# lxa9867/ImageFolder

Hardware: NVIDIA H100
Metric: tokenizer_train_images_per_sec_256x256 (higher is better)
Workload: dtype bf16

## Files before the change

imagefolder_b200/csrc/attn_kernel.cu:

```cuda
#include "xq_common.cuh"
#include "xq_tc.cuh"

namespace xq {
using namespace xqtc;

constexpr int AT_BM = 128;
constexpr int AT_BN = 128;
constexpr int AT_D = 64;
constexpr int AT_NS = 2;
constexpr int AT_TILE = AT_BM * AT_D * 2;
constexpr int AT_THREADS = 288;

struct AttnFwdSmem {
    static constexpr int Q = 0;
    static constexpr int K = AT_TILE;
    static constexpr int V = AT_TILE * (1 + AT_NS);
    static constexpr int BAR = AT_TILE * (1 + 2 * AT_NS);
    static constexpr int BYTES = BAR + 256;
};

__device__ __forceinline__ void named_bar_sync(int id, int nthreads) { asm volatile("bar.sync %0, %1;" ::"r"(id), "r"(nthreads) : "memory"); }

template <typename E>
__global__ void __launch_bounds__(AT_THREADS, 1)
attn_fwd_kernel(const __grid_constant__ CUtensorMap tmQKV, typename E::T *__restrict__ out, float *__restrict__ lse2, int N, int H,
                int nQ , float c ) {
    extern __shared__ uint8_t smem_raw[];
    uint8_t *base = (uint8_t *)(((uintptr_t)smem_raw + 1023) & ~(uintptr_t)1023);
    uint64_t *bars = (uint64_t *)(base + AttnFwdSmem::BAR);
    uint64_t *q_full = bars + 0;
    uint64_t *k_full = bars + 1;
    uint64_t *k_empty = bars + 1 + AT_NS;
    uint64_t *v_full = bars + 1 + 2 * AT_NS;
    uint64_t *v_empty = bars + 1 + 3 * AT_NS;

    const int tid = threadIdx.x, warp = tid >> 5, lane = tid & 31;
    const int nK = (N + AT_BN - 1) / AT_BN;
    const int bh = blockIdx.x / nQ, qt = blockIdx.x - bh * nQ;
    const int b = bh / H, h = bh - b * H;

    if (tid == 0) {
        mbar_init(q_full, 1);
        for (int i = 0; i < AT_NS; ++i) { mbar_init(&k_full[i], 1); mbar_init(&k_empty[i], 8); mbar_init(&v_full[i], 1); mbar_init(&v_empty[i], 8); }
        mbar_fence_init();
    }
    __syncthreads();

    if (warp == 8) {
        const int colQ = h * AT_D, colK = (H + h) * AT_D, colV = (2 * H + h) * AT_D;
        if (elect_one()) {
            tma_prefetch_desc(&tmQKV);
            mbar_expect_tx(q_full, AT_TILE);
            tma_load_3d(base + AttnFwdSmem::Q, &tmQKV, colQ, qt * AT_BM, b, q_full);
        }
        __syncwarp();
        for (int j = 0; j < nK; ++j) {
            const int st = j % AT_NS;
            const uint32_t ph = ((j / AT_NS) & 1) ^ 1;
            mbar_wait(&k_empty[st], ph);
            if (elect_one()) {
                mbar_expect_tx(&k_full[st], AT_TILE);
                tma_load_3d(base + AttnFwdSmem::K + st * AT_TILE, &tmQKV, colK, j * AT_BN, b, &k_full[st]);
            }
            __syncwarp();
            mbar_wait(&v_empty[st], ph);
            if (elect_one()) {
                mbar_expect_tx(&v_full[st], AT_TILE);
                tma_load_3d(base + AttnFwdSmem::V + st * AT_TILE, &tmQKV, colV, j * AT_BN, b, &v_full[st]);
            }
            __syncwarp();
        }
        return;
    }

    const int wg = warp >> 2, wq = warp & 3;
    const int rq = wg * 64 + wq * 16 + (lane >> 2), cq = 2 * (lane & 3);
    const uint64_t qd = desc_k_sw128(smem_u32(base + AttnFwdSmem::Q + wg * (AT_TILE / 2)));
    float m[2] = {-CUDART_INF_F, -CUDART_INF_F}, l[2] = {0.f, 0.f};
    float o[32];
#pragma unroll
    for (int i = 0; i < 32; ++i) o[i] = 0.f;
    mbar_wait(q_full, 0);
    for (int j = 0; j < nK; ++j) {
        const int st = j % AT_NS;
        const uint32_t ph = (j / AT_NS) & 1;
        float s[64];
        mbar_wait(&k_full[st], ph);
        const uint64_t kd = desc_k_sw128(smem_u32(base + AttnFwdSmem::K + st * AT_TILE));
        wgmma_fence();
#pragma unroll
        for (int k = 0; k < AT_D / 16; ++k) wgmma_m64n128k16_ss<E, 0, 0>(s, desc_adv(qd, k * 32), desc_adv(kd, k * 32), (uint32_t)k);
        wgmma_commit();
        wgmma_wait<0>();
        fence_regs(s);
        __syncwarp();
        if (lane == 0) mbar_arrive(&k_empty[st]);
        const int nv = N - j * AT_BN;
        if (nv < AT_BN) {
#pragma unroll
            for (int i = 0; i < 64; ++i)
                if (8 * (i >> 2) + cq + (i & 1) >= nv) s[i] = -CUDART_INF_F;
        }
        float mx[2] = {m[0], m[1]};
#pragma unroll
        for (int i = 0; i < 64; ++i) mx[(i >> 1) & 1] = fmaxf(mx[(i >> 1) & 1], s[i]);
#pragma unroll
        for (int hh = 0; hh < 2; ++hh) {
            mx[hh] = fmaxf(mx[hh], __shfl_xor_sync(0xffffffffu, mx[hh], 1));
            mx[hh] = fmaxf(mx[hh], __shfl_xor_sync(0xffffffffu, mx[hh], 2));
        }
        float alpha[2], mc[2];
#pragma unroll
        for (int hh = 0; hh < 2; ++hh) {
            alpha[hh] = ex2_approx((m[hh] - mx[hh]) * c);
            m[hh] = mx[hh];
            mc[hh] = mx[hh] * c;
            l[hh] *= alpha[hh];
        }
#pragma unroll
        for (int i = 0; i < 32; ++i) o[i] *= alpha[(i >> 1) & 1];
        uint32_t pa[AT_BN / 16][4];
#pragma unroll
        for (int i = 0; i < 64; i += 2) {
            const int hh = (i >> 1) & 1;
            const float p0 = ex2_approx(fmaf(s[i], c, -mc[hh])), p1 = ex2_approx(fmaf(s[i + 1], c, -mc[hh]));
            l[hh] += p0 + p1;
            pa[i >> 3][((i >> 2) & 1) * 2 + hh] = E::pack(p0, p1);
        }
        mbar_wait(&v_full[st], ph);
        const uint64_t vd = desc_mn_sw128(smem_u32(base + AttnFwdSmem::V + st * AT_TILE), AT_TILE);
        wgmma_fence();
#pragma unroll
        for (int k = 0; k < AT_BN / 16; ++k) wgmma_m64n64k16_rs<E, 1>(o, pa[k], desc_adv(vd, k * 2048), 1u);
        wgmma_commit();
        wgmma_wait<0>();
        fence_regs(o);
        __syncwarp();
        if (lane == 0) mbar_arrive(&v_empty[st]);
    }
#pragma unroll
    for (int hh = 0; hh < 2; ++hh) {
        l[hh] += __shfl_xor_sync(0xffffffffu, l[hh], 1);
        l[hh] += __shfl_xor_sync(0xffffffffu, l[hh], 2);
    }
#pragma unroll
    for (int hh = 0; hh < 2; ++hh) {
        const int n = qt * AT_BM + rq + 8 * hh;
        if (n >= N) continue;
        const float inv = 1.0f / l[hh];
        if (cq == 0) lse2[(size_t)bh * N + n] = fmaf(m[hh], c, log2f(l[hh]));
        typename E::T *orow = out + ((size_t)b * N + n) * H * AT_D + h * AT_D;
#pragma unroll
        for (int jj = 0; jj < AT_D / 8; ++jj)
            *reinterpret_cast<uint32_t *>(orow + 8 * jj + cq) = E::pack(o[4 * jj + 2 * hh] * inv, o[4 * jj + 2 * hh + 1] * inv);
    }
}

constexpr int AB_THREADS = 288;
constexpr int AB_BQ = 64;
constexpr int AB_QS = 3;
constexpr int AB_QTILE = AB_BQ * AT_D * 2;

struct AttnBwdSmem {
    static constexpr int K = 0;
    static constexpr int V = AT_TILE;
    static constexpr int Q = 2 * AT_TILE;
    static constexpr int DO = Q + AB_QS * AB_QTILE;
    static constexpr int DS = DO + AB_QS * AB_QTILE;
    static constexpr int STAT = DS + 2 * AB_QTILE;
    static constexpr int BAR = STAT + AB_QS * 512;
    static constexpr int BYTES = BAR + 256;
};

template <typename E>
__device__ __forceinline__ void bwd_epilogue_frag(const float (&acc)[32], float mul, typename E::T *__restrict__ row0,
                                                  size_t row_stride, bool ok0, bool ok1, float *__restrict__ g_bias_cols, int lane) {
    const int cq = 2 * (lane & 3);
#pragma unroll
    for (int jj = 0; jj < AT_D / 8; ++jj) {
        const uint32_t w0 = E::pack(acc[4 * jj] * mul, acc[4 * jj + 1] * mul);
        const uint32_t w1 = E::pack(acc[4 * jj + 2] * mul, acc[4 * jj + 3] * mul);
        if (ok0) *reinterpret_cast<uint32_t *>(row0 + 8 * jj + cq) = w0;
        if (ok1) *reinterpret_cast<uint32_t *>(row0 + 8 * row_stride + 8 * jj + cq) = w1;
        if (g_bias_cols) {
            float s0 = E::lo(w0) + E::lo(w1);
            float s1 = E::hi(w0) + E::hi(w1);
#pragma unroll
            for (int o = 4; o < 32; o <<= 1) {
                s0 += __shfl_xor_sync(0xffffffffu, s0, o);
                s1 += __shfl_xor_sync(0xffffffffu, s1, o);
            }
            if (lane < 4) {
                atomicAdd(g_bias_cols + 8 * jj + cq, s0);
                atomicAdd(g_bias_cols + 8 * jj + cq + 1, s1);
            }
        }
    }
}

template <typename E>
__global__ void __launch_bounds__(AB_THREADS, 1)
attn_bwd_kernel(const __grid_constant__ CUtensorMap tmQKV, const __grid_constant__ CUtensorMap tmDO, const float *__restrict__ lseP,
                const float *__restrict__ deltaP, float *__restrict__ dq_acc, typename E::T *__restrict__ dqkv, float *__restrict__ g_bias,
                int N, int H, int Npad, float c, float scale) {
    extern __shared__ uint8_t smem_raw[];
    uint8_t *base = (uint8_t *)(((uintptr_t)smem_raw + 1023) & ~(uintptr_t)1023);
    uint64_t *bars = (uint64_t *)(base + AttnBwdSmem::BAR);
    uint64_t *kv_full = bars;
    uint64_t *q_full = bars + 1;
    uint64_t *q_empty = bars + 1 + AB_QS;
    float *s_lse = (float *)(base + AttnBwdSmem::STAT);
    float *s_delta = s_lse + AB_QS * AB_BQ;

    const int tid = threadIdx.x, warp = tid >> 5, lane = tid & 31;
    const int bh = blockIdx.y, b = bh / H, h = bh - b * H;
    const int k0 = blockIdx.x * AT_BN;
    const int colQ = h * AT_D, colK = (H + h) * AT_D, colV = (2 * H + h) * AT_D;
    const int nQ = (N + AB_BQ - 1) / AB_BQ;

    if (tid == 0) {
        mbar_init(kv_full, 1);
        for (int i = 0; i < AB_QS; ++i) { mbar_init(&q_full[i], 1); mbar_init(&q_empty[i], 8); }
        mbar_fence_init();
    }
    __syncthreads();

    if (warp == 8) {
        if (elect_one()) {
            tma_prefetch_desc(&tmQKV);
            tma_prefetch_desc(&tmDO);
            mbar_expect_tx(kv_full, 2 * AT_TILE);
            for (int hf = 0; hf < 2; ++hf) {
                tma_load_3d(base + AttnBwdSmem::K + hf * AB_QTILE, &tmQKV, colK, k0 + hf * AB_BQ, b, kv_full);
                tma_load_3d(base + AttnBwdSmem::V + hf * AB_QTILE, &tmQKV, colV, k0 + hf * AB_BQ, b, kv_full);
            }
        }
        __syncwarp();
        for (int i = 0; i < nQ; ++i) {
            const int st = i % AB_QS;
            mbar_wait(&q_empty[st], ((i / AB_QS) & 1) ^ 1);
            if (elect_one()) {
                mbar_expect_tx(&q_full[st], 2 * AB_QTILE + 2 * AB_BQ * 4);
                tma_load_3d(base + AttnBwdSmem::Q + st * AB_QTILE, &tmQKV, colQ, i * AB_BQ, b, &q_full[st]);
                tma_load_3d(base + AttnBwdSmem::DO + st * AB_QTILE, &tmDO, h * AT_D, i * AB_BQ, b, &q_full[st]);
                bulk_g2s(s_lse + st * AB_BQ, lseP + (size_t)bh * Npad + i * AB_BQ, AB_BQ * 4, &q_full[st]);
                bulk_g2s(s_delta + st * AB_BQ, deltaP + (size_t)bh * Npad + i * AB_BQ, AB_BQ * 4, &q_full[st]);
            }
            __syncwarp();
        }
        return;
    }

    const int wg = warp >> 2, wq = warp & 3;
    const int rq = wq * 16 + (lane >> 2), cq = 2 * (lane & 3);
    const int key0 = k0 + wg * 64 + rq;
    const bool kok0 = key0 < N, kok1 = key0 + 8 < N;
    const uint32_t kw = smem_u32(base + AttnBwdSmem::K + wg * AB_QTILE), vw = smem_u32(base + AttnBwdSmem::V + wg * AB_QTILE);
    const uint64_t kd_k = desc_k_sw128(kw), vd_k = desc_k_sw128(vw), kd_mn = desc_mn_sw128(kw, AT_TILE);
    const uint32_t dsw = smem_u32(base + AttnBwdSmem::DS + wg * AB_QTILE);
    const uint64_t dsd = desc_mn_sw128(dsw, AT_TILE);
    float dv[32], dk[32];
#pragma unroll
    for (int i = 0; i < 32; ++i) dv[i] = dk[i] = 0.f;
    mbar_wait(kv_full, 0);
    for (int i = 0; i < nQ; ++i) {
        const int st = i % AB_QS;
        mbar_wait(&q_full[st], (i / AB_QS) & 1);
        const uint32_t qa = smem_u32(base + AttnBwdSmem::Q + st * AB_QTILE), da = smem_u32(base + AttnBwdSmem::DO + st * AB_QTILE);
        float s[32], dp[32];
        wgmma_fence();
#pragma unroll
        for (int k = 0; k < AT_D / 16; ++k) wgmma_m64n64k16_ss<E, 0, 0>(s, desc_adv(kd_k, k * 32), desc_adv(desc_k_sw128(qa), k * 32), (uint32_t)k);
#pragma unroll
        for (int k = 0; k < AT_D / 16; ++k) wgmma_m64n64k16_ss<E, 0, 0>(dp, desc_adv(vd_k, k * 32), desc_adv(desc_k_sw128(da), k * 32), (uint32_t)k);
        wgmma_commit();
        wgmma_wait<0>();
        fence_regs(s);
        fence_regs(dp);
        const float *L = s_lse + st * AB_BQ, *D = s_delta + st * AB_BQ;
        uint32_t pa[4][4], sa[4][4];
#pragma unroll
        for (int jj = 0; jj < AB_BQ / 8; ++jj) {
            const float2 Lq = *reinterpret_cast<const float2 *>(L + 8 * jj + cq);
            const float2 Dq = *reinterpret_cast<const float2 *>(D + 8 * jj + cq);
#pragma unroll
            for (int hh = 0; hh < 2; ++hh) {
                const bool ok = hh ? kok1 : kok0;
                const float p0 = ok ? ex2_approx(fmaf(s[4 * jj + 2 * hh], c, -Lq.x)) : 0.f;
                const float p1 = ok ? ex2_approx(fmaf(s[4 * jj + 2 * hh + 1], c, -Lq.y)) : 0.f;
                const uint32_t pw = E::pack(p0, p1);
                const float d0 = E::lo(pw) * (dp[4 * jj + 2 * hh] - Dq.x);
                const float d1 = E::hi(pw) * (dp[4 * jj + 2 * hh + 1] - Dq.y);
                const uint32_t dw = E::pack(d0, d1);
                pa[jj >> 1][(jj & 1) * 2 + hh] = pw;
                sa[jj >> 1][(jj & 1) * 2 + hh] = dw;
                asm volatile("st.shared.b32 [%0], %1;" ::"r"(dsw + rowtile_off_bf16(rq + 8 * hh, 8 * jj + cq)), "r"(dw) : "memory");
            }
        }
        fence_async_smem();
        named_bar_sync(1 + wg, 128);
        const uint64_t qd_mn = desc_mn_sw128(qa, AT_TILE), dd_mn = desc_mn_sw128(da, AT_TILE);
        float dq[32];
        wgmma_fence();
#pragma unroll
        for (int k = 0; k < AB_BQ / 16; ++k) {
            wgmma_m64n64k16_rs<E, 1>(dv, pa[k], desc_adv(dd_mn, k * 2048), 1u);
            wgmma_m64n64k16_rs<E, 1>(dk, sa[k], desc_adv(qd_mn, k * 2048), 1u);
        }
#pragma unroll
        for (int k = 0; k < 64 / 16; ++k) wgmma_m64n64k16_ss<E, 1, 1>(dq, desc_adv(dsd, k * 2048), desc_adv(kd_mn, k * 2048), (uint32_t)k);
        wgmma_commit();
        wgmma_wait<0>();
        fence_regs(dv);
        fence_regs(dk);
        fence_regs(dq);
        __syncwarp();
        if (lane == 0) mbar_arrive(&q_empty[st]);
        named_bar_sync(1 + wg, 128);
#pragma unroll
        for (int hh = 0; hh < 2; ++hh) {
            const int q = i * AB_BQ + rq + 8 * hh;
            if (q < N) {
                float *dst = dq_acc + ((size_t)bh * N + q) * AT_D + cq;
#pragma unroll
                for (int jj = 0; jj < AT_D / 8; ++jj)
                    atomicAdd(reinterpret_cast<float2 *>(dst + 8 * jj), make_float2(dq[4 * jj + 2 * hh], dq[4 * jj + 2 * hh + 1]));
            }
        }
    }
    const size_t W = (size_t)3 * H * AT_D;
    typename E::T *row = dqkv + ((size_t)b * N + key0) * W;
    bwd_epilogue_frag<E>(dv, 1.0f, row + colV, W, kok0, kok1, g_bias ? g_bias + colV : nullptr, lane);
    bwd_epilogue_frag<E>(dk, scale, row + colK, W, kok0, kok1, g_bias ? g_bias + colK : nullptr, lane);
}


constexpr int AB_KTAIL_MAX = 4;
constexpr int AB_PREP_ROWS = 128;

template <typename E>
__device__ __forceinline__ void unpack8(const uint4 &w, float (&f)[8]) {
    const uint32_t x[4] = {w.x, w.y, w.z, w.w};
#pragma unroll
    for (int e = 0; e < 4; ++e) { f[2 * e] = E::lo(x[e]); f[2 * e + 1] = E::hi(x[e]); }
}

template <typename E, int NT>
__global__ void __launch_bounds__(256, 2)
attn_bwd_prep_kernel(const typename E::T *__restrict__ qkv, const typename E::T *__restrict__ out, const typename E::T *__restrict__ dout,
                     const float *__restrict__ lse2, float *__restrict__ lseP, float *__restrict__ deltaP, float *__restrict__ dq_acc,
                     float *__restrict__ dsT, typename E::T *__restrict__ dqkv, float *__restrict__ g_bias, int N, int H, int Npad,
                     float c, float scale) {
    constexpr int NTA = NT > 0 ? NT : 1;
    __shared__ float red[NT > 0 ? 8 : 1][2][NTA][AT_D];
    __shared__ __align__(16) float skv[2][NTA][AT_D];
    const int bh = blockIdx.y, b = bh / H, h = bh - b * H;
    const int lane = threadIdx.x & 31, sub = threadIdx.x & 7, rloc = threadIdx.x >> 3;
    const int n0 = N - NT;
    const size_t W = (size_t)3 * H * AT_D;
    const typename E::T *qb = qkv + (size_t)b * N * W + h * AT_D + sub * 8;
    const size_t ob = (size_t)b * N * H * AT_D + h * AT_D + sub * 8;
    float aK[NTA][8], aV[NTA][8];
    if constexpr (NT > 0) {
        if (threadIdx.x < NT * 16) {
            const int t = threadIdx.x >> 4, isv = (threadIdx.x >> 3) & 1;
            float f[8];
            unpack8<E>(*reinterpret_cast<const uint4 *>(qb + (size_t)(n0 + t) * W + (size_t)(1 + isv) * H * AT_D), f);
#pragma unroll
            for (int e = 0; e < 8; ++e) skv[isv][t][sub * 8 + e] = f[e];
        }
#pragma unroll
        for (int t = 0; t < NT; ++t) {
#pragma unroll
            for (int e = 0; e < 8; ++e) aK[t][e] = aV[t][e] = 0.f;
        }
        __syncthreads();
    }
    constexpr int PASSES = AB_PREP_ROWS / 32;
    extern __shared__ uint4 prep_stage[];
    auto prefetch = [&](int blk, int stg) {
#pragma unroll
        for (int ps = 0; ps < PASSES; ++ps) {
            const int n = blk * AB_PREP_ROWS + ps * 32 + rloc;
            const int nc = n < N ? n : N - 1;
            uint4 *dst = prep_stage + ((size_t)(stg * 3) * PASSES + ps) * 256 + threadIdx.x;
            cp_async16(dst, out + ob + (size_t)nc * H * AT_D);
            cp_async16(dst + PASSES * 256, dout + ob + (size_t)nc * H * AT_D);
            cp_async16(dst + 2 * PASSES * 256, qb + (size_t)nc * W);
        }
        cp_async_commit();
    };
    if constexpr (NT > 0) prefetch(blockIdx.x, 0);
    int stg = 0;
    for (int blk = blockIdx.x; blk * AB_PREP_ROWS < Npad; blk += gridDim.x, stg ^= 1) {
        uint4 ow[PASSES], gw[PASSES], qw[PASSES];
        float lq[PASSES];
#pragma unroll
        for (int ps = 0; ps < PASSES; ++ps) {
            const int n = blk * AB_PREP_ROWS + ps * 32 + rloc;
            const int nc = n < N ? n : N - 1;
            if constexpr (NT == 0) {
                ow[ps] = *reinterpret_cast<const uint4 *>(out + ob + (size_t)nc * H * AT_D);
                gw[ps] = *reinterpret_cast<const uint4 *>(dout + ob + (size_t)nc * H * AT_D);
            }
            lq[ps] = lse2[(size_t)bh * N + nc];
        }
        if constexpr (NT > 0) {
            if ((blk + (int)gridDim.x) * AB_PREP_ROWS < Npad) { prefetch(blk + gridDim.x, stg ^ 1); cp_async_wait<1>(); }
            else cp_async_wait<0>();
        }
#pragma unroll
        for (int ps = 0; ps < PASSES; ++ps) {
            const int n = blk * AB_PREP_ROWS + ps * 32 + rloc;
            const bool live = n < N;
            float ov[8], gv[8];
            if constexpr (NT > 0) {
                const uint4 *src = prep_stage + ((size_t)(stg * 3) * PASSES + ps) * 256 + threadIdx.x;
                ow[ps] = src[0];
                gw[ps] = src[PASSES * 256];
                qw[ps] = src[2 * PASSES * 256];
            }
            unpack8<E>(ow[ps], ov);
            unpack8<E>(gw[ps], gv);
            float dl = 0.f;
#pragma unroll
            for (int e = 0; e < 8; ++e) dl = fmaf(ov[e], gv[e], dl);
            dl += __shfl_xor_sync(0xffffffffu, dl, 1);
            dl += __shfl_xor_sync(0xffffffffu, dl, 2);
            dl += __shfl_xor_sync(0xffffffffu, dl, 4);
            if (!live) dl = 0.f;
            if (sub == 0) {
                deltaP[(size_t)bh * Npad + n] = dl;
                lseP[(size_t)bh * Npad + n] = live ? lq[ps] : CUDART_INF_F;
            }
            if (live) {
                float4 *z = reinterpret_cast<float4 *>(dq_acc + ((size_t)bh * N + n) * AT_D + sub * 8);
                z[0] = make_float4(0.f, 0.f, 0.f, 0.f);
                z[1] = make_float4(0.f, 0.f, 0.f, 0.f);
            }
            if constexpr (NT > 0) {
                float qv[8];
                unpack8<E>(qw[ps], qv);
#pragma unroll
                for (int t = 0; t < NT; ++t) {
                    float sx = 0.f, pd = 0.f;
                    const float4 k0 = *reinterpret_cast<const float4 *>(&skv[0][t][sub * 8]), k1 = *reinterpret_cast<const float4 *>(&skv[0][t][sub * 8 + 4]);
                    const float4 v0 = *reinterpret_cast<const float4 *>(&skv[1][t][sub * 8]), v1 = *reinterpret_cast<const float4 *>(&skv[1][t][sub * 8 + 4]);
                    const float kt[8] = {k0.x, k0.y, k0.z, k0.w, k1.x, k1.y, k1.z, k1.w}, vt[8] = {v0.x, v0.y, v0.z, v0.w, v1.x, v1.y, v1.z, v1.w};
#pragma unroll
                    for (int e = 0; e < 8; ++e) { sx = fmaf(qv[e], kt[e], sx); pd = fmaf(gv[e], vt[e], pd); }
#pragma unroll
                    for (int o = 4; o > 0; o >>= 1) {
                        sx += __shfl_xor_sync(0xffffffffu, sx, o);
                        pd += __shfl_xor_sync(0xffffffffu, pd, o);
                    }
                    const float p = live ? ex2_approx(fmaf(sx, c, -lq[ps])) : 0.f;
                    const float ds = p * (pd - dl);
#pragma unroll
                    for (int e = 0; e < 8; ++e) { aV[t][e] = fmaf(p, gv[e], aV[t][e]); aK[t][e] = fmaf(ds, qv[e], aK[t][e]); }
                    if (sub == 0 && live) dsT[((size_t)bh * N + n) * NT + t] = ds;
                }
            }
        }
    }
    if constexpr (NT > 0) {
        const int warp = threadIdx.x >> 5;
#pragma unroll
        for (int t = 0; t < NT; ++t) {
#pragma unroll
            for (int e = 0; e < 8; ++e) {
                float a = aK[t][e], v = aV[t][e];
                a += __shfl_xor_sync(0xffffffffu, a, 8);  v += __shfl_xor_sync(0xffffffffu, v, 8);
                a += __shfl_xor_sync(0xffffffffu, a, 16); v += __shfl_xor_sync(0xffffffffu, v, 16);
                if (lane < 8) { red[warp][0][t][sub * 8 + e] = a; red[warp][1][t][sub * 8 + e] = v; }
            }
        }
        __syncthreads();
        if (threadIdx.x < 2 * AT_D) {
            const int which = threadIdx.x / AT_D, d = threadIdx.x - which * AT_D;
            float bsum = 0.f;
#pragma unroll
            for (int t = 0; t < NT; ++t) {
                float sum = 0.f;
#pragma unroll
                for (int w8 = 0; w8 < 8; ++w8) sum += red[w8][which][t][d];
                const typename E::T val = E::from(sum * (which == 0 ? scale : 1.0f));
                dqkv[((size_t)b * N + n0 + t) * W + (size_t)(1 + which) * H * AT_D + h * AT_D + d] = val;
                bsum += E::to(val);
            }
            if (g_bias) atomicAdd(g_bias + (size_t)(1 + which) * H * AT_D + h * AT_D + d, bsum);
        }
    }
}

constexpr int AB_CONV_ROWS = 128;

template <typename E>
__global__ void __launch_bounds__(256)
attn_dq_convert_kernel(const float *__restrict__ dq_acc, const typename E::T *__restrict__ qkv, const float *__restrict__ dsT,
                       typename E::T *__restrict__ dqkv, float *__restrict__ g_bias, int N, int H, int n0, int nt, float scale) {
    __shared__ float red[8][AT_D];
    __shared__ float skt[AB_KTAIL_MAX][AT_D];
    const int part = threadIdx.x & 7, rloc = threadIdx.x >> 3;
    const int bhh = blockIdx.y;
    const int hh = bhh % H, bb = bhh / H;
    constexpr int PASSES = AB_CONV_ROWS / 32;
    float4 x0[PASSES], x1[PASSES];
#pragma unroll
    for (int ps = 0; ps < PASSES; ++ps) {
        const int n = blockIdx.x * AB_CONV_ROWS + ps * 32 + rloc;
        const size_t rowid = (size_t)bhh * N + (n < N ? n : N - 1);
        x0[ps] = *reinterpret_cast<const float4 *>(dq_acc + rowid * AT_D + part * 8);
        x1[ps] = *reinterpret_cast<const float4 *>(dq_acc + rowid * AT_D + part * 8 + 4);
    }
    if (nt > 0) {
        for (int i = threadIdx.x; i < nt * AT_D; i += 256) {
            const int t = i / AT_D, d = i - t * AT_D;
            skt[t][d] = E::to(qkv[(((size_t)bb * N + n0 + t) * 3 * H + H + hh) * AT_D + d]);
        }
        __syncthreads();
    }
    float v[8];
#pragma unroll
    for (int e = 0; e < 8; ++e) v[e] = 0.f;
#pragma unroll
    for (int ps = 0; ps < PASSES; ++ps) {
        const int n = blockIdx.x * AB_CONV_ROWS + ps * 32 + rloc;
        if (n < N) {
            const size_t rowid = (size_t)bhh * N + n;
            float x[8] = {x0[ps].x, x0[ps].y, x0[ps].z, x0[ps].w, x1[ps].x, x1[ps].y, x1[ps].z, x1[ps].w};
            for (int t = 0; t < nt; ++t) {
                const float ds = dsT[rowid * nt + t];
#pragma unroll
                for (int e = 0; e < 8; ++e) x[e] = fmaf(ds, skt[t][part * 8 + e], x[e]);
            }
            uint4 o;
            o.x = E::pack(x[0] * scale, x[1] * scale);
            o.y = E::pack(x[2] * scale, x[3] * scale);
            o.z = E::pack(x[4] * scale, x[5] * scale);
            o.w = E::pack(x[6] * scale, x[7] * scale);
            *reinterpret_cast<uint4 *>(dqkv + (((size_t)bb * N + n) * 3 * H + hh) * AT_D + part * 8) = o;
            const uint32_t w[4] = {o.x, o.y, o.z, o.w};
#pragma unroll
            for (int e = 0; e < 4; ++e) { v[2 * e] += E::lo(w[e]); v[2 * e + 1] += E::hi(w[e]); }
        }
    }
    if (!g_bias) return;
#pragma unroll
    for (int e = 0; e < 8; ++e) {
        v[e] += __shfl_xor_sync(0xffffffffu, v[e], 8);
        v[e] += __shfl_xor_sync(0xffffffffu, v[e], 16);
    }
    const int warp = threadIdx.x >> 5, lane = threadIdx.x & 31;
    if (lane < 8) {
#pragma unroll
        for (int e = 0; e < 8; ++e) red[warp][lane * 8 + e] = v[e];
    }
    __syncthreads();
    if (threadIdx.x < AT_D) {
        float acc = 0.f;
#pragma unroll
        for (int w8 = 0; w8 < 8; ++w8) acc += red[w8][threadIdx.x];
        atomicAdd(g_bias + hh * AT_D + threadIdx.x, acc);
    }
}

static int attn_bwd_ktail(int N) {
    const int r = N % AT_BN;
    return (N > AT_BN && r != 0 && r <= AB_KTAIL_MAX) ? r : 0;
}

static size_t attn_bwd_ws_layout(int B, int N, int H, size_t *off_lse, size_t *off_delta, size_t *off_dst) {
    const size_t Npad = ((size_t)N + AT_BM - 1) / AT_BM * AT_BM;
    const size_t acc = align_up((size_t)B * H * N * AT_D * sizeof(float), 1024);
    const size_t st = align_up((size_t)B * H * Npad * sizeof(float), 1024);
    const size_t dst = align_up((size_t)B * H * N * attn_bwd_ktail(N) * sizeof(float), 1024);
    if (off_lse) *off_lse = acc;
    if (off_delta) *off_delta = acc + st;
    if (off_dst) *off_dst = acc + 2 * st;
    return acc + 2 * st + dst;
}

template <typename E>
static int attn_bwd(const void *qkv, const void *out, const void *d_out, const float *lse2, void *dqkv, float *g_bias, int B, int N,
                    int H, int head_dim, float scale, void *workspace, size_t workspace_bytes, void *stream) {
    using T = typename E::T;
    if (!qkv || !out || !d_out || !lse2 || !dqkv || !workspace || B <= 0 || N <= 0 || H <= 0) return XQ_ERR_ARG;
    if (head_dim != AT_D) return XQ_ERR_UNSUPPORTED;
    if (((uintptr_t)qkv & 15) || ((uintptr_t)out & 15) || ((uintptr_t)d_out & 15) || ((uintptr_t)dqkv & 15) || ((uintptr_t)workspace & 255))
        return XQ_ERR_ARG;
    size_t off_lse, off_delta, off_dst;
    if (workspace_bytes < attn_bwd_ws_layout(B, N, H, &off_lse, &off_delta, &off_dst)) return XQ_ERR_WORKSPACE;
    cudaStream_t st = (cudaStream_t)stream;
    float *acc = (float *)workspace;
    float *lseP = (float *)((char *)workspace + off_lse);
    float *deltaP = (float *)((char *)workspace + off_delta);
    float *dsT = (float *)((char *)workspace + off_dst);
    const uint64_t W = (uint64_t)3 * H * AT_D, Wo = (uint64_t)H * AT_D;
    CUtensorMap tmQKV, tmDO;
    if (!tensor_map_16_3d(&tmQKV, E::TMAP, qkv, W, N, B, W * 2, (uint64_t)N * W * 2, AB_BQ) ||
        !tensor_map_16_3d(&tmDO, E::TMAP, d_out, Wo, N, B, Wo * 2, (uint64_t)N * Wo * 2, AB_BQ))
        return XQ_ERR_UNSUPPORTED;
    const int nt = attn_bwd_ktail(N);
    const int nK = nt ? N / AT_BN : (N + AT_BN - 1) / AT_BN;
    const int Npad = (N + AT_BM - 1) / AT_BM * AT_BM;
    if ((long long)B * H > 65535) return XQ_ERR_UNSUPPORTED;
    if (g_bias) XQ_CUDA_TRY(cudaMemsetAsync(g_bias, 0, (size_t)3 * H * AT_D * sizeof(float), st));
    const float c2 = scale * 1.4426950408889634f;
    {
        dim3 grid(nt ? 1u : (unsigned)(Npad / AB_PREP_ROWS), (unsigned)(B * H));
        const size_t ps = nt ? (size_t)2 * 3 * (AB_PREP_ROWS / 32) * 256 * 16 : 0;
        decltype(&attn_bwd_prep_kernel<E, 0>) const preps[] = {attn_bwd_prep_kernel<E, 0>, attn_bwd_prep_kernel<E, 1>,
                                                               attn_bwd_prep_kernel<E, 2>, attn_bwd_prep_kernel<E, 3>,
                                                               attn_bwd_prep_kernel<E, 4>};
        const auto prep = preps[nt < 4 ? nt : 4];
        if (int rc = smem_optin(prep, ps)) return rc;
        prep<<<grid, 256, ps, st>>>((const T *)qkv, (const T *)out, (const T *)d_out, lse2, lseP, deltaP, acc, dsT, (T *)dqkv, g_bias,
                                    N, H, Npad, c2, scale);
        XQ_LAUNCH_CHECK("attn_bwd_prep_kernel");
    }
    const size_t smem = AttnBwdSmem::BYTES + 1024;
    if (int rc = smem_optin(attn_bwd_kernel<E>, smem)) return rc;
    attn_bwd_kernel<E><<<dim3((unsigned)nK, (unsigned)(B * H)), AB_THREADS, smem, st>>>(tmQKV, tmDO, lseP, deltaP, acc, (T *)dqkv,
                                                                                        g_bias, N, H, Npad, c2, scale);
    XQ_LAUNCH_CHECK("attn_bwd_kernel");
    {
        dim3 grid((unsigned)((N + AB_CONV_ROWS - 1) / AB_CONV_ROWS), (unsigned)(B * H));
        attn_dq_convert_kernel<E><<<grid, 256, 0, st>>>(acc, (const T *)qkv, dsT, (T *)dqkv, g_bias, N, H, N - nt, nt, scale);
        XQ_LAUNCH_CHECK("attn_dq_convert_kernel");
    }
    return XQ_OK;
}

template <typename E>
static int attn_fwd(const void *qkv, void *out, float *lse2, int B, int N, int H, int head_dim, float scale, void *stream) {
    using T = typename E::T;
    if (!qkv || !out || !lse2 || B <= 0 || N <= 0 || H <= 0) return XQ_ERR_ARG;
    if (head_dim != AT_D) return XQ_ERR_UNSUPPORTED;
    if (((uintptr_t)qkv & 15) || ((uintptr_t)out & 15)) return XQ_ERR_ARG;
    const uint64_t W = (uint64_t)3 * H * AT_D;
    CUtensorMap tmQKV;
    if (!tensor_map_16_3d(&tmQKV, E::TMAP, qkv, W, N, B, W * 2, (uint64_t)N * W * 2, AT_BM)) return XQ_ERR_UNSUPPORTED;
    const int nQ = (N + AT_BM - 1) / AT_BM;
    const size_t smem = AttnFwdSmem::BYTES + 1024;
    if (int rc = smem_optin(attn_fwd_kernel<E>, smem)) return rc;
    const long long tiles = (long long)B * H * nQ;
    if (tiles > 0x7fffffffLL) return XQ_ERR_ARG;
    const float c = scale * 1.4426950408889634f;
    attn_fwd_kernel<E><<<(unsigned)tiles, AT_THREADS, smem, (cudaStream_t)stream>>>(tmQKV, (T *)out, lse2, N, H, nQ, c);
    XQ_LAUNCH_CHECK("attn_fwd_kernel");
    return XQ_OK;
}

}

extern "C" {

size_t xq_vit_attn_bwd_workspace_bytes(int B, int N, int H) {
    if (B <= 0 || N <= 0 || H <= 0) return 0;
    return xq::attn_bwd_ws_layout(B, N, H, nullptr, nullptr, nullptr);
}

int xq_vit_attn_bwd(const void *qkv, const void *out, const void *d_out, const float *lse2, void *dqkv, float *g_bias, int B, int N,
                    int H, int head_dim, float scale, void *workspace, size_t workspace_bytes, void *stream) {
    return xq::attn_bwd<xqtc::Bf16>(qkv, out, d_out, lse2, dqkv, g_bias, B, N, H, head_dim, scale, workspace, workspace_bytes, stream);
}
int xq_vit_attn_bwd_f16(const void *qkv, const void *out, const void *d_out, const float *lse2, void *dqkv, float *g_bias, int B,
                        int N, int H, int head_dim, float scale, void *workspace, size_t workspace_bytes, void *stream) {
    return xq::attn_bwd<xqtc::F16>(qkv, out, d_out, lse2, dqkv, g_bias, B, N, H, head_dim, scale, workspace, workspace_bytes, stream);
}

int xq_vit_attn_fwd(const void *qkv, void *out, float *lse2, int B, int N, int H, int head_dim, float scale, void *stream) {
    return xq::attn_fwd<xqtc::Bf16>(qkv, out, lse2, B, N, H, head_dim, scale, stream);
}
int xq_vit_attn_fwd_f16(const void *qkv, void *out, float *lse2, int B, int N, int H, int head_dim, float scale, void *stream) {
    return xq::attn_fwd<xqtc::F16>(qkv, out, lse2, B, N, H, head_dim, scale, stream);
}

}
```

Measured before the change: 642.8.

## Replace per-thread dQ atomics with swizzled smem staging and TMA reduce-add

In the attention backward kernel, each warpgroup now writes its dQ fragment into a double-buffered, 128B-swizzled shared memory tile and issues TMA bulk reduce-add stores to the fp32 dQ accumulator. This replaces per-thread float2 global atomicAdds. The aim is to cut atomic traffic and issue overhead, and to overlap the reduction with the next Q block. It adds shared memory, an extra named barrier per iteration and bulk-wait ordering, plus optional clock instrumentation that is compiled out by default.

```diff
diff --git a/imagefolder_b200/csrc/attn_kernel.cu b/imagefolder_b200/csrc/attn_kernel.cu
--- a/imagefolder_b200/csrc/attn_kernel.cu
+++ b/imagefolder_b200/csrc/attn_kernel.cu
@@ -160,6 +160,11 @@
 constexpr int AB_BQ = 64;
 constexpr int AB_QS = 3;
 constexpr int AB_QTILE = AB_BQ * AT_D * 2;
+constexpr int AB_DQTILE = AB_BQ * AT_D * 4;
+
+__device__ __forceinline__ uint32_t dq_tile_off(int r, int c) {
+    return (uint32_t)((c >> 5) * (AB_DQTILE / 2) + r * 128 + ((((c & 31) >> 2) ^ (r & 7)) << 4) + (c & 3) * 4);
+}
 
 struct AttnBwdSmem {
     static constexpr int K = 0;
@@ -167,10 +172,37 @@
     static constexpr int Q = 2 * AT_TILE;
     static constexpr int DO = Q + AB_QS * AB_QTILE;
     static constexpr int DS = DO + AB_QS * AB_QTILE;
-    static constexpr int STAT = DS + 2 * AB_QTILE;
+    static constexpr int DQ = DS + 2 * AB_QTILE;
+    static constexpr int STAT = DQ + 4 * AB_DQTILE;
     static constexpr int BAR = STAT + AB_QS * 512;
     static constexpr int BYTES = BAR + 256;
 };
+
+enum { AB_CLK_RING, AB_CLK_SCORE_WAIT, AB_CLK_SOFTMAX, AB_CLK_DS_BAR, AB_CLK_GRAD_WAIT, AB_CLK_DQ, AB_CLK_BLOCKS, AB_CLK_SLOTS };
+#ifdef XQ_AB_CLOCKS
+__device__ unsigned long long ab_clocks[AB_CLK_SLOTS];
+struct AbClock {
+    long long t, acc[AB_CLK_SLOTS] = {};
+    bool on;
+    __device__ explicit AbClock(bool on_) : on(on_) {}
+    __device__ void start() { t = clock64(); }
+    __device__ void lap(int slot) { const long long n = clock64(); acc[slot] += n - t; t = n; }
+    __device__ void count(int slot) { ++acc[slot]; }
+    __device__ void flush() {
+        if (!on) return;
+        for (int i = 0; i < AB_CLK_SLOTS; ++i)
+            if (acc[i]) atomicAdd(&ab_clocks[i], (unsigned long long)acc[i]);
+    }
+};
+#else
+struct AbClock {
+    __device__ explicit AbClock(bool) {}
+    __device__ void start() {}
+    __device__ void lap(int) {}
+    __device__ void count(int) {}
+    __device__ void flush() {}
+};
+#endif
 
 template <typename E>
 __device__ __forceinline__ void bwd_epilogue_frag(const float (&acc)[32], float mul, typename E::T *__restrict__ row0,
@@ -200,8 +232,8 @@
 
 template <typename E>
 __global__ void __launch_bounds__(AB_THREADS, 1)
-attn_bwd_kernel(const __grid_constant__ CUtensorMap tmQKV, const __grid_constant__ CUtensorMap tmDO, const float *__restrict__ lseP,
-                const float *__restrict__ deltaP, float *__restrict__ dq_acc, typename E::T *__restrict__ dqkv, float *__restrict__ g_bias,
+attn_bwd_kernel(const __grid_constant__ CUtensorMap tmQKV, const __grid_constant__ CUtensorMap tmDO, const __grid_constant__ CUtensorMap tmDQ,
+                const float *__restrict__ lseP, const float *__restrict__ deltaP, typename E::T *__restrict__ dqkv, float *__restrict__ g_bias,
                 int N, int H, int Npad, float c, float scale) {
     extern __shared__ uint8_t smem_raw[];
     uint8_t *base = (uint8_t *)(((uintptr_t)smem_raw + 1023) & ~(uintptr_t)1023);
@@ -229,6 +261,7 @@
         if (elect_one()) {
             tma_prefetch_desc(&tmQKV);
             tma_prefetch_desc(&tmDO);
+            tma_prefetch_desc(&tmDQ);
             mbar_expect_tx(kv_full, 2 * AT_TILE);
             for (int hf = 0; hf < 2; ++hf) {
                 tma_load_3d(base + AttnBwdSmem::K + hf * AB_QTILE, &tmQKV, colK, k0 + hf * AB_BQ, b, kv_full);
@@ -262,10 +295,15 @@
     float dv[32], dk[32];
 #pragma unroll
     for (int i = 0; i < 32; ++i) dv[i] = dk[i] = 0.f;
+    const bool lead = (tid & 127) == 0;
+    uint8_t *dqt = base + AttnBwdSmem::DQ + wg * 2 * AB_DQTILE;
+    AbClock clk(lead);
     mbar_wait(kv_full, 0);
+    clk.start();
     for (int i = 0; i < nQ; ++i) {
         const int st = i % AB_QS;
         mbar_wait(&q_full[st], (i / AB_QS) & 1);
+        clk.lap(AB_CLK_RING);
         const uint32_t qa = smem_u32(base + AttnBwdSmem::Q + st * AB_QTILE), da = smem_u32(base + AttnBwdSmem::DO + st * AB_QTILE);
         float s[32], dp[32];
         wgmma_fence();
@@ -274,9 +312,11 @@
 #pragma unroll
         for (int k = 0; k < AT_D / 16; ++k) wgmma_m64n64k16_ss<E, 0, 0>(dp, desc_adv(vd_k, k * 32), desc_adv(desc_k_sw128(da), k * 32), (uint32_t)k);
         wgmma_commit();
+        clk.lap(AB_CLK_SOFTMAX);
         wgmma_wait<0>();
         fence_regs(s);
         fence_regs(dp);
+        clk.lap(AB_CLK_SCORE_WAIT);
         const float *L = s_lse + st * AB_BQ, *D = s_delta + st * AB_BQ;
         uint32_t pa[4][4], sa[4][4];
 #pragma unroll
@@ -298,7 +338,9 @@
             }
         }
         fence_async_smem();
+        clk.lap(AB_CLK_SOFTMAX);
         named_bar_sync(1 + wg, 128);
+        clk.lap(AB_CLK_DS_BAR);
         const uint64_t qd_mn = desc_mn_sw128(qa, AT_TILE), dd_mn = desc_mn_sw128(da, AT_TILE);
         float dq[32];
         wgmma_fence();
@@ -310,24 +352,37 @@
 #pragma unroll
         for (int k = 0; k < 64 / 16; ++k) wgmma_m64n64k16_ss<E, 1, 1>(dq, desc_adv(dsd, k * 2048), desc_adv(kd_mn, k * 2048), (uint32_t)k);
         wgmma_commit();
+        clk.lap(AB_CLK_SOFTMAX);
         wgmma_wait<0>();
         fence_regs(dv);
         fence_regs(dk);
         fence_regs(dq);
         __syncwarp();
         if (lane == 0) mbar_arrive(&q_empty[st]);
+        clk.lap(AB_CLK_GRAD_WAIT);
+        if (lead) bulk_wait_read<1>();
         named_bar_sync(1 + wg, 128);
-#pragma unroll
-        for (int hh = 0; hh < 2; ++hh) {
-            const int q = i * AB_BQ + rq + 8 * hh;
-            if (q < N) {
-                float *dst = dq_acc + ((size_t)bh * N + q) * AT_D + cq;
-#pragma unroll
-                for (int jj = 0; jj < AT_D / 8; ++jj)
-                    atomicAdd(reinterpret_cast<float2 *>(dst + 8 * jj), make_float2(dq[4 * jj + 2 * hh], dq[4 * jj + 2 * hh + 1]));
-            }
-        }
-    }
+        clk.lap(AB_CLK_DS_BAR);
+        uint8_t *dqb = dqt + (i & 1) * AB_DQTILE;
+        const uint32_t dqw = smem_u32(dqb);
+#pragma unroll
+        for (int hh = 0; hh < 2; ++hh)
+#pragma unroll
+            for (int jj = 0; jj < AT_D / 8; ++jj)
+                asm volatile("st.shared.v2.f32 [%0], {%1, %2};" ::"r"(dqw + dq_tile_off(rq + 8 * hh, 8 * jj + cq)),
+                             "f"(dq[4 * jj + 2 * hh]), "f"(dq[4 * jj + 2 * hh + 1]) : "memory");
+        fence_async_smem();
+        named_bar_sync(1 + wg, 128);
+        if (lead) {
+            tma_reduce_add_3d(&tmDQ, dqb, 0, i * AB_BQ, bh);
+            tma_reduce_add_3d(&tmDQ, dqb + AB_DQTILE / 2, 32, i * AB_BQ, bh);
+            bulk_commit();
+        }
+        clk.lap(AB_CLK_DQ);
+        clk.count(AB_CLK_BLOCKS);
+    }
+    if (lead) bulk_wait<0>();
+    clk.flush();
     const size_t W = (size_t)3 * H * AT_D;
     typename E::T *row = dqkv + ((size_t)b * N + key0) * W;
     bwd_epilogue_frag<E>(dv, 1.0f, row + colV, W, kok0, kok1, g_bias ? g_bias + colV : nullptr, lane);
@@ -597,9 +652,13 @@
     float *deltaP = (float *)((char *)workspace + off_delta);
     float *dsT = (float *)((char *)workspace + off_dst);
     const uint64_t W = (uint64_t)3 * H * AT_D, Wo = (uint64_t)H * AT_D;
-    CUtensorMap tmQKV, tmDO;
+    CUtensorMap tmQKV, tmDO, tmDQ;
+    const cuuint64_t dq_dims[3] = {(cuuint64_t)AT_D, (cuuint64_t)N, (cuuint64_t)B * H};
+    const cuuint64_t dq_strides[2] = {(cuuint64_t)AT_D * 4, (cuuint64_t)N * AT_D * 4};
+    const cuuint32_t dq_box[3] = {32u, (cuuint32_t)AB_BQ, 1u};
     if (!tensor_map_16_3d(&tmQKV, E::TMAP, qkv, W, N, B, W * 2, (uint64_t)N * W * 2, AB_BQ) ||
-        !tensor_map_16_3d(&tmDO, E::TMAP, d_out, Wo, N, B, Wo * 2, (uint64_t)N * Wo * 2, AB_BQ))
+        !tensor_map_16_3d(&tmDO, E::TMAP, d_out, Wo, N, B, Wo * 2, (uint64_t)N * Wo * 2, AB_BQ) ||
+        !tensor_map(&tmDQ, workspace, CU_TENSOR_MAP_DATA_TYPE_FLOAT32, 3, dq_dims, dq_strides, dq_box, CU_TENSOR_MAP_SWIZZLE_128B))
         return XQ_ERR_UNSUPPORTED;
     const int nt = attn_bwd_ktail(N);
     const int nK = nt ? N / AT_BN : (N + AT_BN - 1) / AT_BN;
@@ -621,7 +680,7 @@
     }
     const size_t smem = AttnBwdSmem::BYTES + 1024;
     if (int rc = smem_optin(attn_bwd_kernel<E>, smem)) return rc;
-    attn_bwd_kernel<E><<<dim3((unsigned)nK, (unsigned)(B * H)), AB_THREADS, smem, st>>>(tmQKV, tmDO, lseP, deltaP, acc, (T *)dqkv,
+    attn_bwd_kernel<E><<<dim3((unsigned)nK, (unsigned)(B * H)), AB_THREADS, smem, st>>>(tmQKV, tmDO, tmDQ, lseP, deltaP, (T *)dqkv,
                                                                                         g_bias, N, H, Npad, c2, scale);
     XQ_LAUNCH_CHECK("attn_bwd_kernel");
     {
@@ -677,4 +736,13 @@
     return xq::attn_fwd<xqtc::F16>(qkv, out, lse2, B, N, H, head_dim, scale, stream);
 }
 
-}
+#ifdef XQ_AB_CLOCKS
+int xq_ab_clocks_read(unsigned long long *out) {
+    XQ_CUDA_TRY(cudaMemcpyFromSymbol(out, xq::ab_clocks, sizeof(xq::ab_clocks)));
+    unsigned long long zero[xq::AB_CLK_SLOTS] = {};
+    XQ_CUDA_TRY(cudaMemcpyToSymbol(xq::ab_clocks, zero, sizeof(zero)));
+    return XQ_OK;
+}
+#endif
+
+}
```

New measurement: 659.3 (median of 6 runs). 1.03x the previous value.
